# rhinempi/Reflexiv

Hardware: AMD Instinct MI355X
Metric: k-mers/sec (extract+count+filter; wall-clock to final contigs beside it) (higher is better)
Workload: dtype u64; 1 GPU; synthetic 5 Gbp in all (5 Gbp per GPU x 1), E.coli-like genome 4640000 bp (1078x), PE150, k=31, -cover 30, 0.5% substitutions; reads_per_gpu=33333334, kmer_instances_per_gpu=4000000080, distinct_kmers=352952250, kmers_kept=4639950, parallelism=1 GPU

## Files before the change

### reflexiv_amd/api.py

```python
from __future__ import annotations

import ctypes as C
from dataclasses import dataclass

import time

import numpy as np

from . import _lib
from ._lib import Params, CRecords, RfxError, TWIN_DS, TWIN_RDD, RFX_OK, RFX_E_CAP


def _p(a):
    return a.ctypes.data_as(C.c_void_p) if a is not None else None


def _cap_error(where, need, detail) -> RfxError:
    e = RfxError(RFX_E_CAP, where, detail)
    e.need = int(need)
    return e


@dataclass
class Records:
# ... 904 lines not shown
        self.text_retries = 0
        while True:
            buf = np.empty(max(cap, 1), np.uint8)
            ln, nc, ntr = C.c_int64(0), C.c_int64(0), C.c_int64(0)
            st = self.L.rfx_sharded_assemble_reads(self.ctx, self.comm, _p(bases), _p(read_off), C.c_int64(n_reads), C.byref(prm),
                                                   generations, C.c_int64(gather_below), _p(buf), C.c_int64(cap), C.byref(ln), C.byref(nc), _p(trace),
                                                   C.c_int64(len(trace)), C.byref(ntr), tot)
            if st == RFX_E_CAP and ln.value > cap:
                cap = int(ln.value)
                self.text_retries += 1
                continue
            self._check(st, "rfx_sharded_assemble_reads")
            return (bytes(buf[:ln.value]).decode(), int(nc.value), [int(x) for x in trace[:ntr.value]], [int(x) for x in tot])

    def comm_bytes_bucketed(self) -> int:
        return int(self.L.rfx_comm_last_bytes_bucketed(self.comm))

    def gather_shards_dev(self, d_keys: int, d_counts: int, n: int, key_words: int, count_bytes: int, root: int,
                          d_out_keys: int, d_out_counts: int, cap: int) -> int:
        m = C.c_int64(0)
        st = self.L.rfx_dev_gather_shards(self.ctx, self.comm, C.c_void_p(d_keys), C.c_void_p(d_counts), C.c_int64(n), key_words,
                                          count_bytes, root, C.c_void_p(d_out_keys), C.c_void_p(d_out_counts), C.c_int64(cap),
                                          C.byref(m))
        if st == RFX_E_CAP:
            e = RfxError(st, "rfx_dev_gather_shards", f"needs room for {m.value} entries, cap is {cap}")
            e.need = int(m.value)
            raise e
        self._check(st, "rfx_dev_gather_shards")
        return int(m.value)

    def count_timing(self):
        out = {}
        for name in ("hist1", "part1", "hist2", "part2", "hist3", "part3", "leaf", "sort", "extract_w", "count_w",
                     "pair_hist", "pair_part", "stat_leaves", "stat_passes", "stat_overflows", "stat_l2_spilled", "stat_l2_void"):
            ms, ln = C.c_float(0), C.c_int64(0)
            if self.L.rfx_last_count_timing(self.ctx, name.encode(), C.byref(ms), C.byref(ln)) == RFX_OK:
                out[name] = (float(ms.value), int(ln.value))
        return out
```

### reflexiv_amd/csrc/rfx_kmer.hip

```cpp
#include "rfx_internal.h"
#include "rfx_device.h"
#include <algorithm>
#include <cmath>
#include <cstdlib>

using namespace rfxd;

namespace {


__device__ __forceinline__ uint64_t nuc_code(uint8_t c) {
    return c == 'A' ? 0 : c == 'C' ? 1 : c == 'G' ? 2 : 3;
}

__global__ void k_encode(const uint8_t *__restrict__ bases, const int64_t *__restrict__ read_off,
                         int64_t n_reads, int wpr, uint64_t *__restrict__ words,
                         uint32_t *__restrict__ read_len) {
    int64_t t = (int64_t)blockIdx.x * blockDim.x + threadIdx.x;
    if (t >= n_reads * wpr) return;
    int64_t r = t / wpr;
    int w = (int)(t % wpr);
    int64_t b0 = read_off[r];
    int64_t len = read_off[r + 1] - b0;
    if (w == 0 && read_len) read_len[r] = (uint32_t)len;
// ... 1283 lines not shown
__global__ void k_reduce_partials(const uint64_t *__restrict__ pk, const uint32_t *__restrict__ pc, int64_t np,
                                  int min_cov, int max_cov, int apply_filter, uint64_t *__restrict__ out_keys,
                                  int32_t *__restrict__ out_counts, unsigned long long cap, CountOut *__restrict__ co,
                                  int pair_out) {
    const int64_t i = (int64_t)blockIdx.x * blockDim.x + threadIdx.x;
    if (i >= np) return;
    const uint64_t key = pk[i];
    if (i > 0 && pk[i - 1] == key) return;
    uint32_t sum = 0;
    for (int64_t j = i; j < np && pk[j] == key; j++) sum += pc[j];
    atomicAdd(&co->n_distinct, 1ULL);
    const int32_t c = (int32_t)sum;
    if (apply_filter && !(c >= min_cov && c <= max_cov)) return;
    const unsigned long long o = atomicAdd(&co->n_out, 1ULL);
    if (o < cap) {
        if (pair_out) ((Rec *)out_keys)[o] = Rec{key, (uint64_t)(uint32_t)c};
        else { out_keys[o] = key; out_counts[o] = c; }
    }
}


constexpr int SK_M = 13;
constexpr int SK_MIN_W = 9;
constexpr int SKT = 1024;

__device__ __forceinline__ uint32_t mmer_key(uint32_t canon) { return __umul24(canon, 0x9E3779u) + canon; }

__device__ __forceinline__ unsigned rec_digit(uint32_t hdr, int used, int bits) {
    return bits ? (unsigned)((hdr << used) >> (32 - bits)) : 0u;
}

template <int W, bool RUNLOOP, int SEG = 16, class F>
__device__ __forceinline__ void seg_runs(const ReadSrc &s, int nk_r, int sgm, const uint64_t (&w)[3], F &&emit,
                                         uint64_t *hi_out, uint64_t *lo_out, uint32_t *wm_lds = nullptr) {
    static_assert(SEG == 16 || SEG == 32, "segment");
    constexpr int PK = SEG;
    constexpr int NM = PK + W - 1;
    static_assert(NM + SK_M - 1 <= 64, "the segment's bases lie in (hi, lo)");
    const int p0 = sgm * PK;
    int v = nk_r - p0;
    v = v > PK ? PK : v;
    if (v <= 0) return;
    const int sh = 2 * ((s.fc + p0) & 31);
    const uint64_t hi = sh ? (w[0] << sh) | (w[1] >> (64 - sh)) : w[0];
    const uint64_t lo = sh ? (w[1] << sh) | (w[2] >> (64 - sh)) : w[1];
    *hi_out = hi; *lo_out = lo;
    constexpr int M2 = 2 * SK_M;
    const uint32_t mmask = (1u << M2) - 1;
    uint32_t val[NM];
    static_assert(SK_M == 13 && NM <= 50, "positions below");
    const uint64_t rhi = revcomp(lo, 32), rlo = revcomp(hi, 32);
    const uint32_t FW[4] = {(uint32_t)(hi >> 32), (uint32_t)hi, (uint32_t)(lo >> 32), (uint32_t)lo};
    const uint32_t RW[4] = {(uint32_t)(rhi >> 32), (uint32_t)rhi, (uint32_t)(rlo >> 32), (uint32_t)rlo};
    auto cut = [&](const uint32_t (&Wd)[4], const int pos) __attribute__((always_inline)) -> uint32_t {
        const int wi = pos >> 4, off = 2 * (pos & 15);
        if (off + M2 <= 32) return (Wd[wi] >> (32 - M2 - off)) & mmask;
        return __builtin_amdgcn_alignbit(Wd[wi], Wd[wi < 3 ? wi + 1 : 3], 32 - off) >> (32 - M2);
    };
#pragma unroll
    for (int j = 0; j < NM; j++) {
        const uint32_t fm = cut(FW, j), rm = cut(RW, 64 - SK_M - j);
        val[j] = mmer_key(fm < rm ? fm : rm);
    }
    uint32_t wm[PK];
    if constexpr (W >= PK - 1) {
#pragma unroll
        for (int j = W - 2; j >= 0; j--) val[j] = val[j] < val[j + 1] ? val[j] : val[j + 1];
#pragma unroll
        for (int j = W + 1; j < NM; j++) val[j] = val[j] < val[j - 1] ? val[j] : val[j - 1];
        wm[0] = val[0];
#pragma unroll
        for (int i = 1; i < PK; i++) wm[i] = val[i] < val[W + i - 1] ? val[i] : val[W + i - 1];
    } else {
        uint32_t sfx[NM], pfx[NM];
#pragma unroll
        for (int j = NM - 1; j >= 0; j--)
            sfx[j] = (j % W == W - 1 || j == NM - 1) ? val[j] : (val[j] < sfx[j + 1] ? val[j] : sfx[j + 1]);
#pragma unroll
        for (int j = 0; j < NM; j++) pfx[j] = (j % W == 0) ? val[j] : (val[j] < pfx[j - 1] ? val[j] : pfx[j - 1]);
#pragma unroll
        for (int i = 0; i < PK; i++) wm[i] = sfx[i] < pfx[i + W - 1] ? sfx[i] : pfx[i + W - 1];
    }
    if constexpr (!RUNLOOP) {
        uint32_t cur = wm[0];
        int start = 0;
#pragma unroll
        for (int i = 1; i < PK; i++) {
            if (i < v && (wm[i] != cur || (PK > 16 && i - start == 16))) {
                emit(start, i - start, cur);
                cur = wm[i]; start = i;
            }
        }
        emit(start, v - start, cur);
        return;
    }
    uint32_t starts = 1u;
#pragma unroll
    for (int i = 1; i < PK; i++) starts |= (uint32_t)(wm[i] != wm[i - 1]) << i;
    starts &= 0xffffffffu >> (32 - v);
    if constexpr (PK > 16) {
        uint32_t cov = starts;
        cov |= cov << 1; cov |= cov << 2; cov |= cov << 4; cov |= cov << 8;
        const uint32_t unc = ~cov & (0xffffffffu >> (32 - v));
        starts |= unc & (0u - unc);
    }
    if (wm_lds) {
#pragma unroll
        for (int i = 0; i < PK; i++) wm_lds[i * SKT + threadIdx.x] = wm[i];
    }
    uint32_t m0 = wm[0], m1 = wm[1], m2 = wm[2], m3 = wm[3], m4 = wm[4], m5 = wm[5], m6 = wm[6], m7 = wm[7], m8 = wm[8],
             m9 = wm[9], m10 = wm[10], m11 = wm[11], m12 = wm[12], m13 = wm[13], m14 = wm[14], m15 = wm[15];
    if (!wm_lds)
        asm("" : "+v"(m0), "+v"(m1), "+v"(m2), "+v"(m3), "+v"(m4), "+v"(m5), "+v"(m6), "+v"(m7), "+v"(m8), "+v"(m9), "+v"(m10),
                 "+v"(m11), "+v"(m12), "+v"(m13), "+v"(m14), "+v"(m15));
    constexpr int UP = PK > 16 ? 16 : 0;
    uint32_t n0 = wm[UP + 0], n1 = wm[UP + 1], n2 = wm[UP + 2], n3 = wm[UP + 3], n4 = wm[UP + 4], n5 = wm[UP + 5], n6 = wm[UP + 6],
             n7 = wm[UP + 7], n8 = wm[UP + 8], n9 = wm[UP + 9], n10 = wm[UP + 10], n11 = wm[UP + 11], n12 = wm[UP + 12],
             n13 = wm[UP + 13], n14 = wm[UP + 14], n15 = wm[UP + 15];
    if (!wm_lds && PK > 16)
        asm("" : "+v"(n0), "+v"(n1), "+v"(n2), "+v"(n3), "+v"(n4), "+v"(n5), "+v"(n6), "+v"(n7), "+v"(n8), "+v"(n9), "+v"(n10),
                 "+v"(n11), "+v"(n12), "+v"(n13), "+v"(n14), "+v"(n15));
    while (starts) {
        const int i0 = __ffs((int)starts) - 1;
        starts &= starts - 1;
        const int i1 = starts ? __ffs((int)starts) - 1 : v;
        uint32_t key;
        if (wm_lds) {
            key = wm_lds[i0 * SKT + threadIdx.x];
        } else {
            const bool b0 = i0 & 1, b1 = i0 & 2, b2 = i0 & 4, b3 = i0 & 8;
            const uint32_t a0 = b0 ? m1 : m0, a1 = b0 ? m3 : m2, a2 = b0 ? m5 : m4, a3 = b0 ? m7 : m6, a4 = b0 ? m9 : m8,
                           a5 = b0 ? m11 : m10, a6 = b0 ? m13 : m12, a7 = b0 ? m15 : m14;
            const uint32_t c0 = b1 ? a1 : a0, c1 = b1 ? a3 : a2, c2 = b1 ? a5 : a4, c3 = b1 ? a7 : a6;
            const uint32_t d0 = b2 ? c1 : c0, d1 = b2 ? c3 : c2;
            key = b3 ? d1 : d0;
            if constexpr (PK > 16) {
                const uint32_t e0 = b0 ? n1 : n0, e1 = b0 ? n3 : n2, e2 = b0 ? n5 : n4, e3 = b0 ? n7 : n6, e4 = b0 ? n9 : n8,
                               e5 = b0 ? n11 : n10, e6 = b0 ? n13 : n12, e7 = b0 ? n15 : n14;
                const uint32_t f0 = b1 ? e1 : e0, f1 = b1 ? e3 : e2, f2 = b1 ? e5 : e4, f3 = b1 ? e7 : e6;
                const uint32_t g0 = b2 ? f1 : f0, g1 = b2 ? f3 : f2;
                const uint32_t ku = b3 ? g1 : g0;
                key = (i0 & 16) ? ku : key;
            }
        }
        emit(i0, i1 - i0, key);
    }
}

__device__ __forceinline__ uint64_t mmer_hash64(uint32_t canon) { return kmer_hash((uint64_t)canon); }

__device__ __forceinline__ unsigned sk_digit(uint32_t canon, const Level &lv) {
    const uint64_t h = mmer_hash64(canon);
    if (lv.n_owners > 0) {
        const unsigned o = (unsigned)__umul64hi(h, (uint64_t)lv.n_owners);
        return lv.sub_bits ? (o << lv.sub_bits) | ((uint32_t)((h << OWNER_BITS) >> 32) >> (32 - lv.sub_bits)) : o;
    }
    return rec_digit((uint32_t)((h << OWNER_BITS) >> 32), 0, lv.bits);
}
// ... 158 lines not shown
        drain(false);
        __syncthreads();
    }
    drain(true);
}
#undef buf
#undef tail
#undef head

constexpr int OSE_MIN = 64, OSE_MAX = 256;
constexpr int OS_CSTRIDE = 16;
constexpr int OS_MAXG = 512;
constexpr int OS_HOLES = 3;
struct OneSweep {
    const uint64_t *reg_start;
    const uint32_t *reg_cap;
    unsigned long long *cursor;
    uint64_t *holes;
    int *overflow;
    uint64_t total;
    unsigned long long *tile_counter;
    uint32_t ose, ose_shift;
};

template <int W, int SEG = 16, bool WIDE = false>
__global__ __launch_bounds__(SKT) void k_sk_sample_hist(ReadSrc s, Level lv, int sample, unsigned long long *__restrict__ hist) {
    __shared__ uint32_t h[1 << MAX_BITS];
    const int nb = 1 << lv.bits;
    for (int i = threadIdx.x; i < nb; i += SKT) h[i] = 0;
    __syncthreads();
    const int64_t ntile = (s.n_threads + SKT - 1) / SKT;
    for (int64_t T = (int64_t)blockIdx.x * sample; T < ntile; T += (int64_t)gridDim.x * sample) {
        const int64_t g = T * SKT + threadIdx.x;
        if (g < s.n_threads) {
            SegPos q;
            q.r = g / s.segs;
            q.sgm = (int)(g - q.r * s.segs);
            uint64_t w[3], hi, lo;
            seg_load<SEG>(s, q, w);
            seg_runs<W, false, SEG>(s, read_nk<WIDE>(s, q.r), q.sgm, w, [&](int, int, uint32_t canon) { atomicAdd(&h[sk_digit(canon, lv)], 1u); }, &hi, &lo);
        }
    }
    __syncthreads();
    for (int i = threadIdx.x; i < nb; i += SKT) if (h[i]) atomicAdd(&hist[i], (unsigned long long)h[i]);
}

__global__ __launch_bounds__(1024) void k_plan_regions(const unsigned long long *__restrict__ hist, int nb, double scale, int G, int cap_pct,
                                                       double tiles,
                                                       uint64_t *__restrict__ reg_start, uint32_t *__restrict__ reg_cap,
                                                       unsigned long long *__restrict__ cursor, unsigned long long *__restrict__ totals) {
    __shared__ uint64_t caps[1 << MAX_BITS];
    __shared__ unsigned long long busiest;
    __shared__ uint32_t ose_s;
    const int d = threadIdx.x;
    if (d == 0) busiest = 0;
    __syncthreads();
    if (d < nb) atomicMax(&busiest, hist[d]);
    __syncthreads();
    if (d == 0) {
        const double per_tile = (double)busiest * scale / tiles;
        ose_s = per_tile <= 16.0 ? 64u : per_tile <= 32.0 ? 128u : per_tile <= 64.0 ? 256u : 0u;
    }
    __syncthreads();
    const uint32_t E = ose_s ? ose_s : OSE_MIN;
    if (d < nb) {
        const double c = (double)hist[d];
        const double est = c * scale;
        double room = (est + 6.0 * scale * sqrt(c + 1.0) + est / 64.0 + 1024.0) * (double)cap_pct / 100.0;
        uint64_t cap = (uint64_t)room + (uint64_t)G * OS_HOLES * E;
        cap = (cap + E - 1) / E * E;
        if (cap > 0xFFFFFF00ULL) cap = 0xFFFFFF00ULL / E * E;
        caps[d] = cap;
        reg_cap[d] = (uint32_t)cap;
    }
// ... 8 lines not shown
    }
}

template <int SEG, bool WIDE> struct OsGeo {
    static constexpr int T = SEG > 16 && !WIDE ? 512 : SKT;
};
template <int W, bool WIDE = false, int SEG = 16>
__global__ __launch_bounds__((OsGeo<SEG, WIDE>::T), WIDE || SEG > 16 ? 4 : 8) void k_sk_onesweep(ReadSrc s, Level lv, OneSweep os,
                                                               std::conditional_t<WIDE, WRec, Rec> *__restrict__ out) {
    using RT = std::conditional_t<WIDE, WRec, Rec>;
    constexpr int SKT = OsGeo<SEG, WIDE>::T;
    extern __shared__ __attribute__((aligned(32))) unsigned char sk_smem[];
    const int nb = 1 << lv.bits;
#define buf ((RT *)sk_smem)
#define tail ((uint32_t *)(sk_smem + (size_t)nb * SKB * sizeof(RT)))
#define head (tail + nb)
#define cstart (tail + 2 * nb)
#define cbase (tail + 3 * nb)
#define nbase (tail + 4 * nb)
#define pbase (tail + 5 * nb)
    constexpr uint32_t DUMP = 0xFFFFFFFFu;
    const uint32_t OSE = os.ose, OSH = os.ose_shift;
    const uint64_t dump_at = os.total - OSE;
    auto grab = [&](int d) __attribute__((always_inline)) -> uint32_t {
        const unsigned long long b = atomicAdd(&os.cursor[(size_t)d * OS_CSTRIDE], (unsigned long long)OSE);
        return b + OSE <= dump_at ? (uint32_t)(b >> OSH) : DUMP;
    };
    auto phys = [&](uint32_t v, uint32_t cs, uint32_t cb, uint32_t nx) __attribute__((always_inline)) -> uint64_t {
        const uint32_t o = v - cs;
        const uint32_t b = o < (uint32_t)OSE ? cb : nx;
        return (b == DUMP ? dump_at : (uint64_t)b << OSH) + (o & (OSE - 1));
    };
    constexpr uint32_t NONE = 0xFFFFFFFEu;
    for (int i = threadIdx.x; i < nb; i += SKT) {
        tail[i] = 0; head[i] = 0; cstart[i] = 0;
        cbase[i] = grab(i);
        nbase[i] = grab(i);
        pbase[i] = grab(i);
    }
    __syncthreads();
    constexpr int LPB = SEG > 16 || WIDE ? 4 : SKB;
    auto drain = [&](bool final) __attribute__((always_inline)) {
#pragma nounroll
        for (int d = threadIdx.x / LPB; d < nb; d += SKT / LPB) {
            const int j = threadIdx.x % LPB;
            const uint32_t h = head[d], t = tail[d], cs = cstart[d], cb = cbase[d], nx = nbase[d];
            uint32_t e, nh;
            if (t - h > (uint32_t)SKB) { e = h + SKB; nh = t; }
            else {
                e = final ? t : (t & ~(uint32_t)(SKA - 1));
                if (e < h) e = h;
                nh = e;
            }
#pragma unroll
            for (int q = 0; q < SKB / LPB; q++) {
                const uint32_t g = h + j + q * LPB;
                if (g < e) out[phys(g, cs, cb, nx)] = buf[(size_t)d * SKB + (g & (SKB - 1))];
            }
            if (j == 0) {
                head[d] = nh;
                if (nh - cs >= (uint32_t)OSE) {
                    uint32_t c = cs, b0 = cb, b1 = nx, b2 = pbase[d];
                    while (nh - c >= (uint32_t)OSE) { c += OSE; b0 = b1; b1 = b2 != NONE ? b2 : grab(d); b2 = NONE; }
                    cstart[d] = c; cbase[d] = b0; nbase[d] = b1; pbase[d] = b2;
                }
            }
        }
    };
    __shared__ long long tile_lds[2];
    const int64_t ntile = (s.n_threads + SKT - 1) / SKT;
    const int my_d = (int)threadIdx.x;
    int64_t T = blockIdx.x;
    for (int rnd = 0; T < ntile; rnd++) {
        long long t_next = 0;
        if (threadIdx.x == SKT - 1) t_next = (long long)gridDim.x + (long long)atomicAdd(os.tile_counter, 1ULL);
        const bool ask = my_d < nb && pbase[my_d] == NONE;
        uint32_t req = DUMP;
        if (ask) req = grab(my_d);
        const int64_t g = T * SKT + threadIdx.x;
        if (g < s.n_threads) {
            SegPos q;
            q.r = g / s.segs;
            q.sgm = (int)(g - q.r * s.segs);
            uint64_t w[3], hi = 0, lo = 0;
            seg_load<SEG>(s, q, w);
            seg_runs<W, true, SEG>(s, read_nk<WIDE>(s, q.r), q.sgm, w, [&](int i0, int n, uint32_t canon) {
                const uint64_t hh = mmer_hash64(canon);
                const uint32_t hdr = (uint32_t)((hh << OWNER_BITS) >> 32);
                const unsigned d = lv.n_owners > 0 ? (((unsigned)__umul64hi(hh, (uint64_t)lv.n_owners) << lv.sub_bits) | (hdr >> (32 - lv.sub_bits)))
                                                   : rec_digit(hdr, 0, lv.bits);
                RT r;
                if constexpr (WIDE) {
                    const uint64_t *gw = s.words + q.r * s.wpr;
                    const int p = s.fc - s.wfl + q.sgm * SEG + i0;
                    const int wi = p >> 5, sft = 2 * (p & 31), last = s.wpr - 1;
                    const uint64_t a0 = gw[wi < last ? wi : last], a1 = gw[wi + 1 < last ? wi + 1 : last];
                    const uint64_t a2 = gw[wi + 2 < last ? wi + 2 : last], a3 = gw[wi + 3 < last ? wi + 3 : last];
                    r.b0 = sft ? (a0 << sft) | (a1 >> (64 - sft)) : a0;
                    r.b1 = sft ? (a1 << sft) | (a2 >> (64 - sft)) : a1;
                    r.b2 = sft ? (a2 << sft) | (a3 >> (64 - sft)) : a2;
                    r.hd = ((uint64_t)(n - 1) << 32) | (uint64_t)hdr;
                } else {
                    const int sft = 2 * i0;
                    r.w0 = sft ? (hi << sft) | (lo >> (64 - sft)) : hi;
                    r.w1 = ((lo << sft) & 0xFFFFFFF000000000ULL) | ((uint64_t)(n - 1) << 32) | (uint64_t)hdr;
                }
                const uint32_t pos = atomicAdd(&tail[d], 1u);
                if (pos - head[d] < (uint32_t)SKB) buf[(size_t)d * SKB + (pos & (SKB - 1))] = r;
                else {
                    const uint32_t cs = cstart[d];
                    if (pos - cs < 2u * OSE) out[phys(pos, cs, cbase[d], nbase[d])] = r;
                    else *os.overflow = 1;
                }
            }, &hi, &lo);
        }
        if (threadIdx.x == SKT - 1) tile_lds[rnd & 1] = t_next;
        if (ask) pbase[my_d] = req;
        __syncthreads();
        drain(false);
        T = tile_lds[rnd & 1];
        __syncthreads();
    }
    drain(true);
    __syncthreads();
    for (int d = threadIdx.x; d < nb; d += SKT) {
        const uint32_t used = tail[d] - cstart[d], cb = cbase[d], nx = nbase[d], px = pbase[d];
        uint64_t *hl = os.holes + ((size_t)d * gridDim.x + blockIdx.x) * OS_HOLES;
        hl[0] = cb != DUMP && used < OSE ? ((((uint64_t)cb << OSH) + used) << 16) | (uint64_t)(OSE - used) : 0;
        hl[1] = nx != DUMP ? (((uint64_t)nx << OSH) << 16) | (uint64_t)OSE : 0;
        hl[2] = px != DUMP && px != NONE ? (((uint64_t)px << OSH) << 16) | (uint64_t)OSE : 0;
    }
}
#undef buf
#undef tail
#undef head
#undef cstart
#undef cbase
#undef nbase
#undef pbase

constexpr int FH_T = 1024;
template <class RT>
__global__ __launch_bounds__(FH_T) void k_fix_holes(OneSweep os, int G, RT *__restrict__ out, uint64_t *__restrict__ seg_begin,
                                                   uint64_t *__restrict__ seg_end, unsigned long long *__restrict__ totals) {
    constexpr int NHMAX = 2048;
    static_assert(NHMAX >= OS_HOLES * OS_MAXG && NHMAX % FH_T == 0, "holes per bucket");
    constexpr int NWMAX = NHMAX * OSE_MAX / 32;
    __shared__ uint32_t hstart[NHMAX], hoff[NHMAX + 1];
    __shared__ uint32_t bitmap[NWMAX];
    __shared__ uint32_t wsum[FH_T / 64];
    const int d = blockIdx.x;
    const int NH = OS_HOLES * G;
    const uint64_t base = os.reg_start[d];
// ... 328 lines not shown
        RCL_PUT(0) RCL_PUT(1) RCL_PUT(2) RCL_PUT(3)
#undef RCL_PUT
        __syncthreads();
        drain(true);
        __syncthreads();
    }
}

constexpr int L2S_STRIDE = 16;
struct L2Plan {
    const uint64_t *seg_begin, *seg_end; const uint64_t *child_start; int *flags;
    void *spill_rec; uint32_t *spill_child; unsigned long long *spill_cursor; uint32_t spill_cap;
    unsigned long long *tail_cursor; uint64_t out_cap;
};
template <int MODE>
__global__ __launch_bounds__(PT) void k_l2_sample(const typename LevelElem<MODE>::T *__restrict__ recs, L2Plan pl, Level lv, int used,
                                                  uint32_t *__restrict__ sampled) {
    __shared__ uint32_t h[1 << MAX_BITS];
    const int p = blockIdx.x, nb = 1 << lv.bits;
    for (int i = threadIdx.x; i < nb; i += PT) h[i] = 0;
    __syncthreads();
    const uint64_t qb = pl.seg_begin[p], qe = pl.seg_end[p];
    for (uint64_t c = (uint64_t)blockIdx.y * L2S_STRIDE; c * PT < qe - qb; c += (uint64_t)gridDim.y * L2S_STRIDE) {
        const uint64_t i = qb + c * PT + threadIdx.x;
        if (i < qe) {
            const typename LevelElem<MODE>::T r = recs[i];
            if constexpr (MODE == 2) { if (r.w1 == 0) continue; }
            atomicAdd(&h[level_digit<MODE>(r, used, lv)], 1u);
        }
    }
    __syncthreads();
    for (int i = threadIdx.x; i < nb; i += PT) if (h[i]) atomicAdd(&sampled[(int64_t)p * nb + i], h[i]);
}
__global__ void k_l2_caps(const uint32_t *__restrict__ sampled, int64_t nchild, uint32_t *__restrict__ ccap, int pct) {
    const int64_t c = (int64_t)blockIdx.x * blockDim.x + threadIdx.x;
    if (c >= nchild) return;
    const float s = (float)sampled[c];
    uint32_t C = (uint32_t)((float)L2S_STRIDE * (s + 6.0f * sqrtf(s + 1.0f) + 32.0f));
    if (pct != 100) C = (uint32_t)((uint64_t)C * (uint64_t)pct / 100u);
    ccap[c] = (C + 7u) & ~7u;
}
__global__ __launch_bounds__(1024) void k_l2_check(L2Plan pl, int nseg, int64_t nchild, uint64_t out_cap) {
    __shared__ unsigned long long sum_n, mx_n;
    if (threadIdx.x == 0) { sum_n = 0; mx_n = 0; }
    __syncthreads();
    if ((int)threadIdx.x < nseg) {
        const unsigned long long n = pl.seg_end[threadIdx.x] - pl.seg_begin[threadIdx.x];
        atomicAdd(&sum_n, n);
        atomicMax(&mx_n, n);
    }
    __syncthreads();
    if (threadIdx.x == 0) {
        const unsigned long long mean = sum_n / (unsigned long long)(nseg > 0 ? nseg : 1);
        pl.flags[0] = (pl.child_start[nchild] + 8ULL * pl.spill_cap + 65536ULL > out_cap || mx_n > mean + mean / 2 + 4096) ? 1 : 0;
        pl.flags[1] = 0;
        *pl.spill_cursor = 0;
        *pl.tail_cursor = (pl.child_start[nchild] + 7ULL) & ~7ULL;
    }
}

template <int B, int MODE>
__global__ __launch_bounds__(WCT) void k_rec_l2sweep(const typename LevelElem<MODE>::T *__restrict__ recs, L2Plan pl, Level lv, int used,
                                                     typename LevelElem<MODE>::T *__restrict__ out, uint64_t *__restrict__ leaf_end) {
    using Rec = typename LevelElem<MODE>::T;
    extern __shared__ __attribute__((aligned(32))) unsigned char wc_smem[];
    constexpr int A = B / 2;
    if (pl.flags[0]) return;
    const int p = blockIdx.x;
    const int nb = 1 << lv.bits;
    const uint64_t qb = pl.seg_begin[p], qe = pl.seg_end[p];
    Rec *buf = (Rec *)wc_smem;
    unsigned long long *tail = (unsigned long long *)(buf + (size_t)nb * B);
    unsigned long long *head = tail + nb;
    unsigned long long *lim = head + nb;
    for (int i = threadIdx.x; i < nb; i += WCT) {
        tail[i] = head[i] = pl.child_start[(int64_t)p * nb + i];
        lim[i] = pl.child_start[(int64_t)p * nb + i + 1];
    }
    __syncthreads();
    auto drain = [&](bool final) __attribute__((always_inline)) {
#pragma nounroll
        for (int d = threadIdx.x / B; d < nb; d += WCT / B) {
            const int j = threadIdx.x % B;
            const unsigned long long h = head[d], lm = lim[d];
            unsigned long long t = tail[d];
            if (t > lm) t = lm;
            unsigned long long e, nh;
            if (t - h > (unsigned long long)B) { e = h + B; nh = t; }
            else {
                e = final ? t : (t & ~(unsigned long long)(A - 1));
                if (e < h) e = h;
                nh = e;
            }
            const unsigned long long g = h + j;
            if (g < e) out[g] = buf[(size_t)d * B + (g & (B - 1))];
            if (j == 0) head[d] = nh;
        }
    };
    for (uint64_t b0 = qb; b0 < qe; b0 += (uint64_t)WCT * WC_PER) {
        Rec r[WC_PER];
#pragma unroll
        for (int i = 0; i < WC_PER; i++) {
            const uint64_t idx = b0 + (uint64_t)i * WCT + threadIdx.x;
            r[i] = recs[idx < qe ? idx : qe - 1];
        }
#pragma unroll
        for (int i = 0; i < WC_PER; i++) {
            const uint64_t idx = b0 + (uint64_t)i * WCT + threadIdx.x;
            bool live = idx < qe;
            if constexpr (MODE == 2) live = live && r[i].w1 != 0;
            if (live) {
                const unsigned d = level_digit<MODE>(r[i], used, lv);
                const unsigned long long g = atomicAdd(&tail[d], 1ULL);
                if (g >= lim[d]) {
                    const unsigned long long sk = atomicAdd(pl.spill_cursor, 1ULL);
                    if (sk < (unsigned long long)pl.spill_cap) { ((Rec *)pl.spill_rec)[sk] = r[i]; pl.spill_child[sk] = (uint32_t)(p * nb + (int)d); }
                    else pl.flags[1] = 1;
                }
                else if (g - head[d] < (unsigned long long)B) buf[(size_t)d * B + (g & (B - 1))] = r[i];
                else out[g] = r[i];
            }
        }
        __syncthreads();
        drain(false);
        __syncthreads();
    }
    drain(true);
    __syncthreads();
    for (int d = threadIdx.x; d < nb; d += WCT) leaf_end[(int64_t)p * nb + d] = tail[d];
}

constexpr int L2F_T = 1024, L2F_SLOTS = 2048, L2F_MAXC = 1536;
template <class RT>
__global__ __launch_bounds__(L2F_T) void k_l2_spill_fix(L2Plan pl, uint64_t *__restrict__ cstart, uint64_t *__restrict__ lend, RT *__restrict__ out) {
    __shared__ uint32_t tkey[L2F_SLOTS], tcnt[L2F_SLOTS], tfill[L2F_SLOTS], tcap[L2F_SLOTS];
    __shared__ unsigned long long tbase[L2F_SLOTS];
    __shared__ uint32_t ndistinct;
    __shared__ int bad;
    if (pl.flags[0] || pl.flags[1]) return;
    const unsigned long long ns = *pl.spill_cursor;
    if (ns == 0) return;
    constexpr uint32_t NOKEY = 0xFFFFFFFFu;
    for (int i = threadIdx.x; i < L2F_SLOTS; i += L2F_T) { tkey[i] = NOKEY; tcnt[i] = 0; tfill[i] = 0; }
    if (threadIdx.x == 0) { ndistinct = 0; bad = 0; }
    __syncthreads();
    auto find = [&](uint32_t c, bool insert) __attribute__((always_inline)) -> int {
        uint32_t slot = (c * 0x9E3779B1u) >> 21;
        for (int probe = 0; probe < L2F_SLOTS; probe++) {
            uint32_t k = tkey[slot];
            if (k == c) return (int)slot;
            if (k == NOKEY) {
                if (!insert) return -1;
                k = atomicCAS(&tkey[slot], NOKEY, c);
                if (k == NOKEY) { atomicAdd(&ndistinct, 1u); return (int)slot; }
                if (k == c) return (int)slot;
            }
            slot = (slot + 1) & (L2F_SLOTS - 1);
        }
        return -1;
// ... 805 lines not shown
                RFX_HIP(hipFuncSetAttribute((const void *)k_sk_onesweep<19, true>, hipFuncAttributeMaxDynamicSharedMemorySize, (int)lds));
                hipLaunchKernelGGL((k_sk_onesweep<19, true>), dim3((unsigned)G), dim3(SKT), lds, ctx->stream, rsrc, lv, os, dst);
            }
        } else {
            switch (W) {
#define X(w) case w: if (seg32) { \
                         RFX_HIP(hipFuncSetAttribute((const void *)k_sk_onesweep<w, false, 32>, hipFuncAttributeMaxDynamicSharedMemorySize, (int)lds)); \
                         hipLaunchKernelGGL((k_sk_onesweep<w, false, 32>), dim3((unsigned)G), dim3(OST), lds, ctx->stream, rsrc, lv, os, dst); \
                     } else { \
                         RFX_HIP(hipFuncSetAttribute((const void *)k_sk_onesweep<w>, hipFuncAttributeMaxDynamicSharedMemorySize, (int)lds)); \
                         hipLaunchKernelGGL((k_sk_onesweep<w>), dim3((unsigned)G), dim3(SKT), lds, ctx->stream, rsrc, lv, os, dst); \
                     } break;
                RFX_SK_W_CASES(X)
                default: X(19)
#undef X
            }
        }
        RFX_HIP(hipGetLastError());
        hipLaunchKernelGGL(k_fix_holes<Rec>, dim3((unsigned)nb), dim3(FH_T), 0, ctx->stream, os, G, dst, d_seg_begin, d_seg_end,
                           totals.as<unsigned long long>());
        RFX_HIP(hipGetLastError());
    }
    int h_over = 0;
    RFX_HIP(hipMemcpyAsync(h_tot, totals.p, 16, hipMemcpyDeviceToHost, ctx->stream));
    RFX_HIP(hipMemcpyAsync(&h_over, d_overflow, 4, hipMemcpyDeviceToHost, ctx->stream));
    RFX_TRY(sync_checked(ctx));
    if (getenv("RFX_TRACE"))
        fprintf(stderr, "one-sweep level 1: %llu records in regions of %llu (sample 1/%d, %d workgroups, extents of %u)%s\n", h_tot[1], h_tot[0], sample, G, ose,
                h_over ? " -- a region overflowed: two passes instead" : "");
    if (h_over == 2) { ctx->last_error = "one-sweep level 1: holes and tail records do not balance"; return RFX_E_STATE; }
    if (h_over) return RFX_OK;
    *out_recs = dst;
    *n_recs = (int64_t)h_tot[1];
    *done = true;
    return RFX_OK;
}

template <int MODE>
static int records_resweep(rfx_ctx *ctx, const typename LevelElem<MODE>::T *recs, int64_t n_recs, const Level &lv, int used, int oslot,
                           uint64_t *d_seg_begin, uint64_t *d_seg_end, const typename LevelElem<MODE>::T **out_recs, bool *done,
                           const char *hn, const char *pn) {
    using RT = typename LevelElem<MODE>::T;
    *done = false;
    const int mode = getenv("RFX_REC_ONESWEEP") ? atoi(getenv("RFX_REC_ONESWEEP")) : (MODE == 0 || MODE == 3 ? 1 : 0);
    if (MODE == 2 || !mode || lv.bits < 4 || lv.bits > 9 || lv.n_owners > 0 || (mode != 2 && n_recs < ((int64_t)1 << 24))) return RFX_OK;
    const int nb = 1 << lv.bits;
    constexpr int B = MODE == 3 ? 8 : 16;
    if (nb > 256 && B * sizeof(RT) * nb + 28 * (size_t)nb > 160 * 1024) return RFX_OK;
    const size_t lds = (size_t)nb * (B * sizeof(RT) + 28);
    const int64_t nchunk = ceil_div(n_recs, PT);
    int sample = 32;
    if (nchunk < 256 * (int64_t)sample) sample = (int)std::max<int64_t>(1, nchunk / 256);
    const int64_t n_sampled = ceil_div(nchunk, sample);
    DevBuf hist, reg_start, cursor;
    RFX_HIP(hist.alloc((size_t)nb * 8 + 8, ctx->stream));
    RFX_HIP(reg_start.alloc((size_t)(nb + 1) * 8, ctx->stream));
    RFX_HIP(cursor.alloc((size_t)nb * 8, ctx->stream));
    RFX_HIP(hipMemsetAsync(hist.p, 0, (size_t)nb * 8 + 8, ctx->stream));
    const ClaimPlan pl{reg_start.as<uint64_t>(), cursor.as<unsigned long long>(), (int *)(hist.as<unsigned long long>() + nb)};
    {
        ScopedTimer t(ctx, hn);
        hipLaunchKernelGGL(k_rec_sample_hist<MODE>, dim3((unsigned)std::min<int64_t>(n_sampled, (int64_t)ctx->num_cu * 8)), dim3(PT), 0, ctx->stream,
                           recs, (uint64_t)n_recs, lv, used, sample, hist.as<unsigned long long>());
        RFX_HIP(hipGetLastError());
        hipLaunchKernelGGL(k_claim_plan, dim3(1), dim3(1024), 0, ctx->stream, (const unsigned long long *)hist.as<unsigned long long>(), nb,
                           (double)nchunk / (double)n_sampled, pl);
// ... 139 lines not shown
template <int MODE>
static int last_level_sweep(rfx_ctx *ctx, const typename LevelElem<MODE>::T *cur_h, int64_t n_recs, int slot, int bits_last, int used_h,
                            const uint64_t *sb, const uint64_t *seg_end, int64_t nseg_h, size_t level_index,
                            const typename LevelElem<MODE>::T **dst_out, DevBuf &cstart, DevBuf &lend, int64_t *nchild_out, uint64_t *total_out,
                            bool *ok) {
    using RT = typename LevelElem<MODE>::T;
    *ok = false;
    const bool l2s_off = getenv("RFX_L2_ONESWEEP") && atoi(getenv("RFX_L2_ONESWEEP")) == 0;
    const int nb = 1 << bits_last;
    if (l2s_off || bits_last < 4 || bits_last > 10 || nseg_h > 1024 || n_recs < (int64_t)nseg_h * nb * 256) return RFX_OK;
    const int64_t nchild = nseg_h << bits_last;
    const uint32_t spill_cap = (uint32_t)std::min<int64_t>((int64_t)1 << 22, std::max<int64_t>(65536, n_recs / 256));
    const uint64_t bound = (uint64_t)n_recs * 2 + (uint64_t)nchild * 640 + 4096 + 8ULL * spill_cap + 65536;
    const int oslot = slot == 0 ? 1 : 0;
    RT *dst = (RT *)ctx->ws_get(oslot, (size_t)bound * sizeof(RT));
    if (!dst) { ctx->last_error = "workspace allocation failed"; return RFX_E_HIP; }
    DevBuf sampled, ccap, flags, spill_rec, spill_child;
    RFX_HIP(spill_rec.alloc((size_t)spill_cap * sizeof(RT), ctx->stream));
    RFX_HIP(spill_child.alloc((size_t)spill_cap * 4, ctx->stream));
    RFX_HIP(sampled.alloc((size_t)nchild * 4, ctx->stream)); RFX_HIP(ccap.alloc((size_t)nchild * 4, ctx->stream));
    RFX_HIP(cstart.alloc((size_t)(nchild + 1) * 8, ctx->stream));
    RFX_HIP(flags.alloc(32, ctx->stream));
    RFX_HIP(lend.alloc((size_t)nchild * 8, ctx->stream));
    RFX_HIP(hipMemsetAsync(sampled.p, 0, (size_t)nchild * 4, ctx->stream));
    L2Plan pl{sb, seg_end ? seg_end : sb + 1, (const uint64_t *)cstart.as<uint64_t>(), flags.as<int>(), spill_rec.p, spill_child.as<uint32_t>(),
              flags.as<unsigned long long>() + 1, spill_cap, flags.as<unsigned long long>() + 2, bound};
    Level lv{};
    lv.bits = bits_last;
    {
        ScopedTimer t(ctx, level_index == 0 ? "hist1" : level_index == 1 ? "hist2" : "hist3");
        hipLaunchKernelGGL(k_l2_sample<MODE>, dim3((unsigned)nseg_h, 8), dim3(PT), 0, ctx->stream, cur_h, pl, lv, used_h, sampled.as<uint32_t>());
        RFX_HIP(hipGetLastError());
        hipLaunchKernelGGL(k_l2_caps, dim3((unsigned)ceil_div(nchild, 256)), dim3(256), 0, ctx->stream, (const uint32_t *)sampled.as<uint32_t>(), nchild,
                           ccap.as<uint32_t>(), getenv("RFX_L2_SQUEEZE") ? std::max(1, atoi(getenv("RFX_L2_SQUEEZE"))) : 100);
        RFX_HIP(hipGetLastError());
    }
    RFX_TRY(exclusive_scan_u32_to_u64(ctx, ccap.as<uint32_t>(), cstart.as<uint64_t>(), nchild));
    {
        ScopedTimer t(ctx, level_index == 0 ? "part1" : level_index == 1 ? "part2" : "part3");
        hipLaunchKernelGGL(k_l2_check, dim3(1), dim3(1024), 0, ctx->stream, pl, (int)nseg_h, nchild, bound);
        RFX_HIP(hipGetLastError());
        constexpr int B9 = MODE == 3 ? 8 : 16, B10 = B9 / 2;
        if (bits_last <= 9) {
            const size_t lds = (size_t)nb * (B9 * sizeof(RT) + 24);
            RFX_HIP(hipFuncSetAttribute((const void *)k_rec_l2sweep<B9, MODE>, hipFuncAttributeMaxDynamicSharedMemorySize, (int)lds));
            hipLaunchKernelGGL((k_rec_l2sweep<B9, MODE>), dim3((unsigned)nseg_h), dim3(WCT), lds, ctx->stream, cur_h, pl, lv, used_h, dst, lend.as<uint64_t>());
        } else {
            const size_t lds = (size_t)nb * (B10 * sizeof(RT) + 24);
            RFX_HIP(hipFuncSetAttribute((const void *)k_rec_l2sweep<B10, MODE>, hipFuncAttributeMaxDynamicSharedMemorySize, (int)lds));
            hipLaunchKernelGGL((k_rec_l2sweep<B10, MODE>), dim3((unsigned)nseg_h), dim3(WCT), lds, ctx->stream, cur_h, pl, lv, used_h, dst, lend.as<uint64_t>());
        }
        RFX_HIP(hipGetLastError());
        hipLaunchKernelGGL(k_l2_spill_fix<RT>, dim3(1), dim3(L2F_T), 0, ctx->stream, pl, cstart.as<uint64_t>(), lend.as<uint64_t>(), dst);
        RFX_HIP(hipGetLastError());
    }
    unsigned long long h_fl[3] = {0, 0, 0};
    uint64_t h_tot = 0;
    RFX_HIP(hipMemcpyAsync(h_fl, flags.p, 24, hipMemcpyDeviceToHost, ctx->stream));
    RFX_HIP(hipMemcpyAsync(&h_tot, cstart.as<uint64_t>() + nchild, 8, hipMemcpyDeviceToHost, ctx->stream));
    RFX_TRY(sync_checked(ctx));
    const int h_flags[2] = {(int)(h_fl[0] & 0xffffffffULL), (int)(h_fl[0] >> 32)};
    if (!h_flags[0] && !h_flags[1]) ctx->timing["stat_l2_spilled"].launches += (int64_t)h_fl[1];
    if (!h_flags[0] && h_flags[1]) ctx->timing["stat_l2_void"].launches += 1;
    if (getenv("RFX_TRACE")) {
        fprintf(stderr, "last level in one sweep: %lld records in regions of %llu%s\n", (long long)n_recs, (unsigned long long)h_tot,
                h_flags[0] ? " -- not tried (skew, or no room): the exact form instead" : h_flags[1] ? " -- more spilled than the list takes: the exact form instead" : "");
        if (!h_flags[0] && !h_flags[1] && h_fl[1])
// ... 3 lines not shown
        std::vector<uint64_t> hs((size_t)nchild + 1), he((size_t)nchild);
        std::vector<uint32_t> hsm((size_t)nchild);
        RFX_HIP(hipMemcpy(hs.data(), cstart.p, hs.size() * 8, hipMemcpyDeviceToHost));
        RFX_HIP(hipMemcpy(he.data(), lend.p, he.size() * 8, hipMemcpyDeviceToHost));
        RFX_HIP(hipMemcpy(hsm.data(), sampled.p, hsm.size() * 4, hipMemcpyDeviceToHost));
        int64_t nover = 0; double worst = 0; int64_t wi = 0;
        for (int64_t c = 0; c < nchild; c++) {
            const uint64_t capc = hs[(size_t)c + 1] - hs[(size_t)c], need = he[(size_t)c] - hs[(size_t)c];
            if (need > capc) { nover++; const double r = (double)need / (double)capc; if (r > worst) { worst = r; wi = c; } }
        }
        {
            int64_t z = 0, r2 = 0, r4 = 0, big = 0;
            for (int64_t c = 0; c < nchild; c++) {
                const uint64_t need = he[(size_t)c] - hs[(size_t)c];
                if (need > hs[(size_t)c + 1] - hs[(size_t)c]) {
                    if (hsm[(size_t)c] == 0) z++;
                    else { const double r = (double)need / (16.0 * hsm[(size_t)c]); if (r > 4) r4++; else if (r > 2) r2++; }
                    if (need > 4000) big++;
                }
            }
            fprintf(stderr, "  of the children that ran over: %lld with nothing sampled, %lld with need > 4 x estimate, %lld with 2-4 x; %lld hold > 4000 records\n",
                    (long long)z, (long long)r4, (long long)r2, (long long)big);
            std::vector<uint64_t> hb((size_t)nseg_h), hen((size_t)nseg_h);
            RFX_HIP(hipMemcpy(hb.data(), sb, hb.size() * 8, hipMemcpyDeviceToHost));
            RFX_HIP(hipMemcpy(hen.data(), seg_end ? seg_end : sb + 1, hen.size() * 8, hipMemcpyDeviceToHost));
            uint64_t mn = ~0ULL, mx = 0;
            for (int64_t q = 0; q < nseg_h; q++) { const uint64_t n = hen[(size_t)q] - hb[(size_t)q]; mn = std::min(mn, n); mx = std::max(mx, n); }
            fprintf(stderr, "  parents: %lld of %llu .. %llu records\n", (long long)nseg_h, (unsigned long long)mn, (unsigned long long)mx);
        }
        fprintf(stderr, "  %lld of %lld children ran over; worst: child %lld sampled %u, region %llu, holds %llu\n", (long long)nover, (long long)nchild,
                (long long)wi, hsm[(size_t)wi], (unsigned long long)(hs[(size_t)wi + 1] - hs[(size_t)wi]), (unsigned long long)(he[(size_t)wi] - hs[(size_t)wi]));
    }
    if (h_flags[0] || h_flags[1]) return RFX_OK;
    *dst_out = dst; *nchild_out = nchild; *total_out = bound; *ok = true;
    return RFX_OK;
}

template <int MODE>
static int partition_to_leaves(rfx_ctx *ctx, const typename LevelElem<MODE>::T *recs, int64_t n_recs, int ws_slot_of_recs,
                               const std::vector<int> &bits, size_t first_level, int used, DevBuf *seg_cur, DevBuf *seg_next, int64_t nseg,
                               const uint64_t *seg_end_first, const typename LevelElem<MODE>::T **cur_out, int64_t *elem_count,
                               const uint64_t **leaf_off, const uint64_t **leaf_end, int64_t *nleaf, DevBuf &cstart, DevBuf &lend) {
    using RT = typename LevelElem<MODE>::T;
    *leaf_end = nullptr;
    if (bits.size() <= first_level) {
        *cur_out = recs; *elem_count = n_recs; *leaf_off = (const uint64_t *)seg_cur->as<uint64_t>(); *nleaf = nseg;
        *leaf_end = seg_end_first;
        return RFX_OK;
    }
    const size_t last = bits.size() - 1;
    std::vector<int> head(bits.begin(), bits.begin() + (long)last);
    int slot = ws_slot_of_recs, used_h = used;
    const RT *cur_h = recs;
    int64_t nseg_h = nseg;
    DevBuf *sc = seg_cur, *sn = seg_next;
    const uint64_t *seg_end = seg_end_first;
    DevBuf seg_end_head;
    if (last > first_level) {
        RFX_TRY(partition_record_levels<MODE>(ctx, recs, n_recs, ws_slot_of_recs, head, first_level, used, &sc, &sn, &nseg_h, &cur_h, seg_end_first,
                                              &seg_end_head, &seg_end));
        for (size_t l = first_level; l < last; l++) { used_h += bits[l]; slot = slot == 0 ? 1 : 0; }
    }
    bool ok = false;
    const RT *dst = nullptr;
    int64_t nchild = 0;
    uint64_t total = 0;
// ... 787 lines not shown
```

Measured before the change: 197.4 billion k-mers/s.

## Prefetch next tile in scatter and L2 sweep loops, rescale L2 child caps

The superkmer scatter kernel now claims its next tile one round earlier through a three-slot LDS ring and loads that tile's segment words before the drain barrier, so global load latency overlaps the drain. The L2 sweep kernel is restructured to load the next tile of records as 16-byte vectors while the current tile is scattered. The L2 cap kernel now scales each sampled count by how many records the sampler actually saw in that parent instead of a fixed stride, which should tighten allocations and reduce spills. A counter for swept L2 passes is added. The cost is more live registers and the risk of a wrong cap estimate.

```diff
diff --git a/reflexiv_amd/api.py b/reflexiv_amd/api.py
--- a/reflexiv_amd/api.py
+++ b/reflexiv_amd/api.py
@@ -960,7 +960,8 @@
     def count_timing(self):
         out = {}
         for name in ("hist1", "part1", "hist2", "part2", "hist3", "part3", "leaf", "sort", "extract_w", "count_w",
-                     "pair_hist", "pair_part", "stat_leaves", "stat_passes", "stat_overflows", "stat_l2_spilled", "stat_l2_void"):
+                     "pair_hist", "pair_part", "stat_leaves", "stat_passes", "stat_overflows", "stat_l2_spilled", "stat_l2_void",
+                     "stat_l2_swept"):
             ms, ln = C.c_float(0), C.c_int64(0)
             if self.L.rfx_last_count_timing(self.ctx, name.encode(), C.byref(ms), C.byref(ln)) == RFX_OK:
                 out[name] = (float(ms.value), int(ln.value))
diff --git a/reflexiv_amd/csrc/rfx_kmer.hip b/reflexiv_amd/csrc/rfx_kmer.hip
--- a/reflexiv_amd/csrc/rfx_kmer.hip
+++ b/reflexiv_amd/csrc/rfx_kmer.hip
@@ -1737,6 +1737,8 @@
         return (b == DUMP ? dump_at : (uint64_t)b << OSH) + (o & (OSE - 1));
     };
     constexpr uint32_t NONE = 0xFFFFFFFEu;
+    __shared__ long long tile_lds[3];
+    if (threadIdx.x == SKT - 1) tile_lds[1] = (long long)gridDim.x + (long long)atomicAdd(os.tile_counter, 1ULL);
     for (int i = threadIdx.x; i < nb; i += SKT) {
         tail[i] = 0; head[i] = 0; cstart[i] = 0;
         cbase[i] = grab(i);
@@ -1772,23 +1774,30 @@
             }
         }
     };
-    __shared__ long long tile_lds[2];
     const int64_t ntile = (s.n_threads + SKT - 1) / SKT;
     const int my_d = (int)threadIdx.x;
+    SegPos q{0, 0};
+    uint64_t w[3];
+    bool have = false;
+    auto fetch = [&](int64_t tile) __attribute__((always_inline)) {
+        const int64_t g = tile * SKT + threadIdx.x;
+        have = g < s.n_threads;
+        if (have) {
+            q.r = g / s.segs;
+            q.sgm = (int)(g - q.r * s.segs);
+            seg_load<SEG>(s, q, w);
+        }
+    };
     int64_t T = blockIdx.x;
+    fetch(T);
     for (int rnd = 0; T < ntile; rnd++) {
         long long t_next = 0;
         if (threadIdx.x == SKT - 1) t_next = (long long)gridDim.x + (long long)atomicAdd(os.tile_counter, 1ULL);
         const bool ask = my_d < nb && pbase[my_d] == NONE;
         uint32_t req = DUMP;
         if (ask) req = grab(my_d);
-        const int64_t g = T * SKT + threadIdx.x;
-        if (g < s.n_threads) {
-            SegPos q;
-            q.r = g / s.segs;
-            q.sgm = (int)(g - q.r * s.segs);
-            uint64_t w[3], hi = 0, lo = 0;
-            seg_load<SEG>(s, q, w);
+        if (have) {
+            uint64_t hi = 0, lo = 0;
             seg_runs<W, true, SEG>(s, read_nk<WIDE>(s, q.r), q.sgm, w, [&](int i0, int n, uint32_t canon) {
                 const uint64_t hh = mmer_hash64(canon);
                 const uint32_t hdr = (uint32_t)((hh << OWNER_BITS) >> 32);
@@ -1819,11 +1828,12 @@
                 }
             }, &hi, &lo);
         }
-        if (threadIdx.x == SKT - 1) tile_lds[rnd & 1] = t_next;
+        if (threadIdx.x == SKT - 1) tile_lds[(rnd + 2) % 3] = t_next;
         if (ask) pbase[my_d] = req;
+        T = tile_lds[(rnd + 1) % 3];
+        fetch(T);
         __syncthreads();
         drain(false);
-        T = tile_lds[rnd & 1];
         __syncthreads();
     }
     drain(true);
@@ -2218,11 +2228,17 @@
     __syncthreads();
     for (int i = threadIdx.x; i < nb; i += PT) if (h[i]) atomicAdd(&sampled[(int64_t)p * nb + i], h[i]);
 }
-__global__ void k_l2_caps(const uint32_t *__restrict__ sampled, int64_t nchild, uint32_t *__restrict__ ccap, int pct) {
+__global__ void k_l2_caps(const uint32_t *__restrict__ sampled, int64_t nchild, uint32_t *__restrict__ ccap, int pct, L2Plan pl, int bits) {
     const int64_t c = (int64_t)blockIdx.x * blockDim.x + threadIdx.x;
     if (c >= nchild) return;
     const float s = (float)sampled[c];
-    uint32_t C = (uint32_t)((float)L2S_STRIDE * (s + 6.0f * sqrtf(s + 1.0f) + 32.0f));
+    const int64_t p = c >> bits;
+    const uint64_t n = pl.seg_end[p] - pl.seg_begin[p];
+    const uint64_t chunks = (n + PT - 1) / PT, ns = (chunks + L2S_STRIDE - 1) / L2S_STRIDE;
+    uint64_t seen = ns * PT;
+    if (ns && (ns - 1) * L2S_STRIDE == chunks - 1) seen -= chunks * PT - n;
+    const float scale = seen ? (float)n / (float)seen : (float)L2S_STRIDE;
+    uint32_t C = (uint32_t)(scale * (s + 6.0f * sqrtf(s + 1.0f)) + (float)L2S_STRIDE * 32.0f);
     if (pct != 100) C = (uint32_t)((uint64_t)C * (uint64_t)pct / 100u);
     ccap[c] = (C + 7u) & ~7u;
 }
@@ -2283,34 +2299,50 @@
             if (j == 0) head[d] = nh;
         }
     };
-    for (uint64_t b0 = qb; b0 < qe; b0 += (uint64_t)WCT * WC_PER) {
-        Rec r[WC_PER];
-#pragma unroll
-        for (int i = 0; i < WC_PER; i++) {
-            const uint64_t idx = b0 + (uint64_t)i * WCT + threadIdx.x;
-            r[i] = recs[idx < qe ? idx : qe - 1];
-        }
-#pragma unroll
-        for (int i = 0; i < WC_PER; i++) {
-            const uint64_t idx = b0 + (uint64_t)i * WCT + threadIdx.x;
-            bool live = idx < qe;
-            if constexpr (MODE == 2) live = live && r[i].w1 != 0;
-            if (live) {
-                const unsigned d = level_digit<MODE>(r[i], used, lv);
-                const unsigned long long g = atomicAdd(&tail[d], 1ULL);
-                if (g >= lim[d]) {
-                    const unsigned long long sk = atomicAdd(pl.spill_cursor, 1ULL);
-                    if (sk < (unsigned long long)pl.spill_cap) { ((Rec *)pl.spill_rec)[sk] = r[i]; pl.spill_child[sk] = (uint32_t)(p * nb + (int)d); }
-                    else pl.flags[1] = 1;
-                }
-                else if (g - head[d] < (unsigned long long)B) buf[(size_t)d * B + (g & (B - 1))] = r[i];
-                else out[g] = r[i];
-            }
-        }
+    constexpr uint64_t TILE = (uint64_t)WCT * WC_PER;
+    using V = ulonglong2;
+    constexpr int NV = sizeof(Rec) / 16;
+    static_assert(NV == 1 || NV == 2, "16- or 32-byte records");
+    static_assert(WC_PER == 4, "four named records below");
+    V q0, q1, q2, q3, w0 = {}, w1 = {}, w2 = {}, w3 = {};
+#define L2S_LOAD(i, b0) { const uint64_t idx = (b0) + (uint64_t)(i) * WCT + threadIdx.x; const uint64_t at = (idx < qe ? idx : qe - 1) * NV; \
+        q##i = ((const V *)recs)[at]; if constexpr (NV == 2) w##i = ((const V *)recs)[at + 1]; }
+#define L2S_LOAD_TILE(b0) if ((b0) < qe) { L2S_LOAD(0, b0) L2S_LOAD(1, b0) L2S_LOAD(2, b0) L2S_LOAD(3, b0) }
+    auto put = [&](Rec *base, unsigned long long at, const V a, const V b2) __attribute__((always_inline)) {
+        V *to = (V *)base + at * NV;
+        to[0] = a;
+        if constexpr (NV == 2) to[1] = b2;
+    };
+    auto digit_of = [&](const V a, const V b2) __attribute__((always_inline)) -> unsigned {
+        if constexpr (NV == 2) return level_digit<MODE>(Rec{a.x, a.y, b2.x, b2.y}, used, lv);
+        else return level_digit<MODE>(Rec{a.x, a.y}, used, lv);
+    };
+#define L2S_PUT(i) { const uint64_t idx = b0 + (uint64_t)(i) * WCT + threadIdx.x; \
+        bool live = idx < qe; \
+        if constexpr (MODE == 2) live = live && q##i.y != 0; \
+        const unsigned d = digit_of(q##i, w##i); \
+        asm volatile("" : : "v"(d)); \
+        if (live) { \
+            const unsigned long long g = atomicAdd(&tail[d], 1ULL); \
+            if (g >= lim[d]) {                                  \
+                const unsigned long long sk = atomicAdd(pl.spill_cursor, 1ULL); \
+                if (sk < (unsigned long long)pl.spill_cap) { put((Rec *)pl.spill_rec, sk, q##i, w##i); pl.spill_child[sk] = (uint32_t)(p * nb + (int)d); } \
+                else pl.flags[1] = 1;                           \
+            } \
+            else if (g - head[d] < (unsigned long long)B) put(buf, (unsigned long long)d * B + (g & (B - 1)), q##i, w##i); \
+            else put(out, g, q##i, w##i); \
+        } }
+    L2S_LOAD_TILE(qb)
+    for (uint64_t b0 = qb; b0 < qe; b0 += TILE) {
+        L2S_PUT(0) L2S_PUT(1) L2S_PUT(2) L2S_PUT(3)
+        L2S_LOAD_TILE(b0 + TILE)
         __syncthreads();
         drain(false);
         __syncthreads();
     }
+#undef L2S_PUT
+#undef L2S_LOAD_TILE
+#undef L2S_LOAD
     drain(true);
     __syncthreads();
     for (int d = threadIdx.x; d < nb; d += WCT) leaf_end[(int64_t)p * nb + d] = tail[d];
@@ -3387,7 +3419,7 @@
         hipLaunchKernelGGL(k_l2_sample<MODE>, dim3((unsigned)nseg_h, 8), dim3(PT), 0, ctx->stream, cur_h, pl, lv, used_h, sampled.as<uint32_t>());
         RFX_HIP(hipGetLastError());
         hipLaunchKernelGGL(k_l2_caps, dim3((unsigned)ceil_div(nchild, 256)), dim3(256), 0, ctx->stream, (const uint32_t *)sampled.as<uint32_t>(), nchild,
-                           ccap.as<uint32_t>(), getenv("RFX_L2_SQUEEZE") ? std::max(1, atoi(getenv("RFX_L2_SQUEEZE"))) : 100);
+                           ccap.as<uint32_t>(), getenv("RFX_L2_SQUEEZE") ? std::max(1, atoi(getenv("RFX_L2_SQUEEZE"))) : 100, pl, bits_last);
         RFX_HIP(hipGetLastError());
     }
     RFX_TRY(exclusive_scan_u32_to_u64(ctx, ccap.as<uint32_t>(), cstart.as<uint64_t>(), nchild));
@@ -3457,6 +3489,7 @@
                 (long long)wi, hsm[(size_t)wi], (unsigned long long)(hs[(size_t)wi + 1] - hs[(size_t)wi]), (unsigned long long)(he[(size_t)wi] - hs[(size_t)wi]));
     }
     if (h_flags[0] || h_flags[1]) return RFX_OK;
+    ctx->timing["stat_l2_swept"].launches += 1;
     *dst_out = dst; *nchild_out = nchild; *total_out = bound; *ok = true;
     return RFX_OK;
 }
```

Measured after the change: 198.3 billion k-mers/s, median of 6. Within noise of the previous version (+0.4%).

## Merge super-k-mer runs across adjacent 32-base segments via wavefront shuffles

Applied to the files above, without the earlier changes.

For 32-wide segments, neighbouring lanes exchange their head and tail minimizers and boundary run positions through shuffles. A run that continues across a segment boundary is extended into the next segment's bases and the duplicate start is removed there, so fewer super-k-mer records are emitted and partitioned. The record packing borrows the next segment's leading bases so an extended run still encodes its k-mers. Inactive tail threads now take part in the shuffles, and the merge adds cross-lane logic that depends on adjacent lanes holding consecutive segments of the same read.

```diff
diff --git a/reflexiv_amd/api.py b/reflexiv_amd/api.py
--- a/reflexiv_amd/api.py
+++ b/reflexiv_amd/api.py
@@ -960,7 +960,7 @@
     def count_timing(self):
         out = {}
         for name in ("hist1", "part1", "hist2", "part2", "hist3", "part3", "leaf", "sort", "extract_w", "count_w",
-                     "pair_hist", "pair_part", "stat_leaves", "stat_passes", "stat_overflows", "stat_l2_spilled", "stat_l2_void"):
+                     "pair_hist", "pair_part", "stat_leaves", "stat_passes", "stat_overflows", "stat_l2_spilled", "stat_l2_void", "stat_records"):
             ms, ln = C.c_float(0), C.c_int64(0)
             if self.L.rfx_last_count_timing(self.ctx, name.encode(), C.byref(ms), C.byref(ln)) == RFX_OK:
                 out[name] = (float(ms.value), int(ln.value))
diff --git a/reflexiv_amd/csrc/rfx_kmer.hip b/reflexiv_amd/csrc/rfx_kmer.hip
--- a/reflexiv_amd/csrc/rfx_kmer.hip
+++ b/reflexiv_amd/csrc/rfx_kmer.hip
@@ -1339,15 +1339,20 @@
 
 template <int W, bool RUNLOOP, int SEG = 16, class F>
 __device__ __forceinline__ void seg_runs(const ReadSrc &s, int nk_r, int sgm, const uint64_t (&w)[3], F &&emit,
-                                         uint64_t *hi_out, uint64_t *lo_out, uint32_t *wm_lds = nullptr) {
+                                         uint64_t *hi_out, uint64_t *lo_out, uint32_t *wm_lds = nullptr, uint32_t *nx_out = nullptr) {
     static_assert(SEG == 16 || SEG == 32, "segment");
     constexpr int PK = SEG;
+    constexpr bool MERGE = SEG == 32;
+    static_assert(!MERGE || RUNLOOP, "the merged cut walks the run-start bits");
     constexpr int NM = PK + W - 1;
     static_assert(NM + SK_M - 1 <= 64, "the segment's bases lie in (hi, lo)");
     const int p0 = sgm * PK;
     int v = nk_r - p0;
     v = v > PK ? PK : v;
-    if (v <= 0) return;
+    if constexpr (MERGE) {
+        v = v < 0 ? 0 : v;
+        if (!__any(v > 0)) return;
+    } else if (v <= 0) return;
     const int sh = 2 * ((s.fc + p0) & 31);
     const uint64_t hi = sh ? (w[0] << sh) | (w[1] >> (64 - sh)) : w[0];
     const uint64_t lo = sh ? (w[1] << sh) | (w[2] >> (64 - sh)) : w[1];
@@ -1404,12 +1409,33 @@
     uint32_t starts = 1u;
 #pragma unroll
     for (int i = 1; i < PK; i++) starts |= (uint32_t)(wm[i] != wm[i - 1]) << i;
-    starts &= 0xffffffffu >> (32 - v);
+    const uint32_t vmask = v ? 0xffffffffu >> (32 - v) : 0u;
+    starts &= vmask;
     if constexpr (PK > 16) {
         uint32_t cov = starts;
         cov |= cov << 1; cov |= cov << 2; cov |= cov << 4; cov |= cov << 8;
-        const uint32_t unc = ~cov & (0xffffffffu >> (32 - v));
+        const uint32_t unc = ~cov & vmask;
         starts |= unc & (0u - unc);
+    }
+    int vend = v;
+    if constexpr (MERGE) {
+        const int lane = (int)(threadIdx.x & 63);
+        const uint32_t rest = starts & (starts - 1);
+        const int b = !v ? 0 : rest ? __ffs((int)rest) - 1 : v;
+        const int t = v == PK ? __clz((int)starts) + 1 : 0;
+        const uint32_t hk = wm[0], tk = wm[PK - 1];
+        const uint32_t hk_n = (uint32_t)__shfl_down((int)hk, 1);
+        const uint32_t pk_n = (uint32_t)__shfl_down((int)(((uint32_t)(lo >> 32) & 0xFFFFFFC0u) | (uint32_t)b), 1);
+        const uint32_t tk_p = (uint32_t)__shfl_up((int)tk, 1);
+        const int t_p = __shfl_up(t, 1);
+        const bool next_same = lane < 63 && sgm + 1 < s.segs, prev_same = lane > 0 && sgm > 0;
+        const int b_n = (int)(pk_n & 31u);
+        if (nx_out) *nx_out = next_same ? pk_n & 0xFFFFFFC0u : 0u;
+        if (next_same && t > 0 && b_n > 0 && tk == hk_n) vend = v + (16 - t < b_n ? 16 - t : b_n);
+        if (prev_same && t_p > 0 && b > 0 && tk_p == hk) {
+            const int a = 16 - t_p < b ? 16 - t_p : b;
+            if (a > 0) starts = (starts & ~1u) | (a < b ? 1u << a : 0u);
+        }
     }
     if (wm_lds) {
 #pragma unroll
@@ -1430,7 +1456,7 @@
     while (starts) {
         const int i0 = __ffs((int)starts) - 1;
         starts &= starts - 1;
-        const int i1 = starts ? __ffs((int)starts) - 1 : v;
+        const int i1 = starts ? __ffs((int)starts) - 1 : vend;
         uint32_t key;
         if (wm_lds) {
             key = wm_lds[i0 * SKT + threadIdx.x];
@@ -1655,14 +1681,18 @@
     const int64_t ntile = (s.n_threads + SKT - 1) / SKT;
     for (int64_t T = (int64_t)blockIdx.x * sample; T < ntile; T += (int64_t)gridDim.x * sample) {
         const int64_t g = T * SKT + threadIdx.x;
-        if (g < s.n_threads) {
-            SegPos q;
+        const bool in = g < s.n_threads;
+        SegPos q{0, 0};
+        int nk_r = 0;
+        uint64_t w[3] = {0, 0, 0}, hi, lo;
+        if (in) {
             q.r = g / s.segs;
             q.sgm = (int)(g - q.r * s.segs);
-            uint64_t w[3], hi, lo;
             seg_load<SEG>(s, q, w);
-            seg_runs<W, false, SEG>(s, read_nk<WIDE>(s, q.r), q.sgm, w, [&](int, int, uint32_t canon) { atomicAdd(&h[sk_digit(canon, lv)], 1u); }, &hi, &lo);
-        }
+            nk_r = read_nk<WIDE>(s, q.r);
+        }
+        if (SEG == 32 || in)
+            seg_runs<W, SEG == 32, SEG>(s, nk_r, q.sgm, w, [&](int, int, uint32_t canon) { atomicAdd(&h[sk_digit(canon, lv)], 1u); }, &hi, &lo);
     }
     __syncthreads();
     for (int i = threadIdx.x; i < nb; i += SKT) if (h[i]) atomicAdd(&hist[i], (unsigned long long)h[i]);
@@ -1783,13 +1813,19 @@
         uint32_t req = DUMP;
         if (ask) req = grab(my_d);
         const int64_t g = T * SKT + threadIdx.x;
-        if (g < s.n_threads) {
-            SegPos q;
+        const bool in = g < s.n_threads;
+        SegPos q{0, 0};
+        int nk_r = 0;
+        uint64_t w[3] = {0, 0, 0}, hi = 0, lo = 0;
+        uint32_t past = 0;
+        if (in) {
             q.r = g / s.segs;
             q.sgm = (int)(g - q.r * s.segs);
-            uint64_t w[3], hi = 0, lo = 0;
             seg_load<SEG>(s, q, w);
-            seg_runs<W, true, SEG>(s, read_nk<WIDE>(s, q.r), q.sgm, w, [&](int i0, int n, uint32_t canon) {
+            nk_r = read_nk<WIDE>(s, q.r);
+        }
+        if (SEG == 32 || in) {
+            seg_runs<W, true, SEG>(s, nk_r, q.sgm, w, [&](int i0, int n, uint32_t canon) {
                 const uint64_t hh = mmer_hash64(canon);
                 const uint32_t hdr = (uint32_t)((hh << OWNER_BITS) >> 32);
                 const unsigned d = lv.n_owners > 0 ? (((unsigned)__umul64hi(hh, (uint64_t)lv.n_owners) << lv.sub_bits) | (hdr >> (32 - lv.sub_bits)))
@@ -1807,8 +1843,9 @@
                     r.hd = ((uint64_t)(n - 1) << 32) | (uint64_t)hdr;
                 } else {
                     const int sft = 2 * i0;
+                    const uint64_t x = (uint64_t)past << 32;
                     r.w0 = sft ? (hi << sft) | (lo >> (64 - sft)) : hi;
-                    r.w1 = ((lo << sft) & 0xFFFFFFF000000000ULL) | ((uint64_t)(n - 1) << 32) | (uint64_t)hdr;
+                    r.w1 = ((sft ? (lo << sft) | (x >> (64 - sft)) : lo) & 0xFFFFFFF000000000ULL) | ((uint64_t)(n - 1) << 32) | (uint64_t)hdr;
                 }
                 const uint32_t pos = atomicAdd(&tail[d], 1u);
                 if (pos - head[d] < (uint32_t)SKB) buf[(size_t)d * SKB + (pos & (SKB - 1))] = r;
@@ -1817,7 +1854,7 @@
                     if (pos - cs < 2u * OSE) out[phys(pos, cs, cbase[d], nbase[d])] = r;
                     else *os.overflow = 1;
                 }
-            }, &hi, &lo);
+            }, &hi, &lo, nullptr, &past);
         }
         if (threadIdx.x == SKT - 1) tile_lds[rnd & 1] = t_next;
         if (ask) pbase[my_d] = req;
@@ -3182,6 +3219,7 @@
     if (h_over) return RFX_OK;
     *out_recs = dst;
     *n_recs = (int64_t)h_tot[1];
+    ctx->timing["stat_records"].launches += (int64_t)h_tot[1];
     *done = true;
     return RFX_OK;
 }
```

Result: faster. 193.6 billion k-mers/s before, 198.5 billion k-mers/s after, median of 6 (+2.5%).
